# rvp-group/srrg2_proslam

Hardware: AMD Instinct MI355X
Metric: tracked frames/sec on KITTI-00 stereo (1241x376, ~2k kp); SE(3) vs ref (higher is better)
Workload: dtype u64 popcount (Hamming) + f32 (projection, Jacobians, 6x6 normal equations)

## Files before the change

srrg2_proslam_amd/csrc/align.hip:

```cpp
#include "prs_device.h"
#include "prs_host.h"
#include "prs_se3.h"

#include <math.h>
#include <string.h>

#include <type_traits>
#include <vector>

namespace prs {

constexpr int kAlignThreads = 256;
constexpr int kTerms        = 29;
constexpr uint32_t kNoneU32 = 0xffffffffu;
constexpr float kFltMax     = 3.402823466e+38f;

typedef unsigned int au32x4 __attribute__((ext_vector_type(4)));

struct AlignShared {
  float X[16];
  float A[16];
  float Sinv[16];
  float T[16];
  float Tprev[16];
// ... 383 lines not shown
  const double sx = (double) st[0], sy = (double) st[1];
  mean[0]          = (float) (sx / (16.0 * dn));
  mean[1]          = (float) (sy / (16.0 * dn));
  const double cxx = ((double) st[2] - sx * sx / dn) / dn / 256.0;
  const double cxy = ((double) st[3] - sx * sy / dn) / dn / 256.0;
  const double cyy = ((double) st[4] - sy * sy / dn) / dn / 256.0;
  const double half_diff = 0.5 * (cxx - cyy);
  double lambda          = 0.5 * (cxx + cyy) + sqrt(half_diff * half_diff + cxy * cxy);
  if (!(lambda > 0.0)) {
    lambda = 0.0;
  }
  double vx = lambda - cyy, vy = cxy;
  const double norm = sqrt(vx * vx + vy * vy);
  if (norm > 0.0) {
    vx = vx / norm;
    vy = vy / norm;
  } else {
    vx = cxx >= cyy ? 1.0 : 0.0;
    vy = cxx >= cyy ? 0.0 : 1.0;
  }
  normal[0] = (float) vx;
  normal[1] = (float) vy;
  return n < min_points || 3.0 * sqrt(lambda) < leaf_range;
}
__device__ __forceinline__ float kd_side(const KdNode& nd, const float x, const float y) {
  const float dx = x - nd.mx, dy = y - nd.my;
  return dx * nd.nx + dy * nd.ny;
}
__host__ __device__ __forceinline__ int kd_open_capacity(const int max_fixed) {
  return max_fixed / 5 + 4;
}

template <int T, bool SPLIT, int STYPE, int SLOTS = 4>
__global__ __launch_bounds__(T, SPLIT ? 6 : 1) void align_kernel(const AlignArgs g) {
  extern __shared__ __attribute__((aligned(16))) unsigned char smem[];
  const int tid   = threadIdx.x;
  const int lane  = tid & 63;
  const int wave  = tid >> 6;
  const int tid_hot = tid;
  constexpr bool kReuse = SPLIT && SLOTS == 4;
  const int frame = blockIdx.x;

  int nF = g.b.n_fixed[frame];
  int nM = g.b.n_moving[frame];
  nF     = nF < 0 ? 0 : (nF > g.b.fixed_stride ? g.b.fixed_stride : nF);
  nM     = nM < 0 ? 0 : (nM > g.b.moving_stride ? g.b.moving_stride : nM);
  const size_t fbase = (size_t) frame * (size_t) g.b.fixed_stride;
  const size_t mbase = (size_t) frame * (size_t) g.b.moving_stride;
  const float4* __restrict__ gfix = reinterpret_cast<const float4*>(g.b.fixed) + fbase;
  const float4* __restrict__ gmov = reinterpret_cast<const float4*>(g.b.moving) + mbase;
  const au32x4* __restrict__ gfd  = reinterpret_cast<const au32x4*>(g.b.fixed_desc + fbase * PRS_DESC_BYTES);
  const au32x4* __restrict__ gmd  = reinterpret_cast<const au32x4*>(g.b.moving_desc + mbase * PRS_DESC_BYTES);
  prs_corr* __restrict__ gcorr    = g.b.corr + fbase;
  prs_pcf_state* gstate           = g.b.state + frame;
  prs_align_result* gres          = g.b.result + frame;

  uint2* db           = reinterpret_cast<uint2*>(smem + g.off_db);
  uint16_t* inv       = reinterpret_cast<uint16_t*>(smem + g.off_inv);
  uint16_t* cellstart = reinterpret_cast<uint16_t*>(smem + g.off_cellstart);
  float4* cfix        = reinterpret_cast<float4*>(smem + g.off_cfix);
  float4* cmov        = reinterpret_cast<float4*>(smem + g.off_cmov);
  au32x4* fdesc       = reinterpret_cast<au32x4*>(smem + g.off_fdesc);
  au32x4* fdesc_hi    = fdesc + g.max_fixed;
  float2* fuv         = reinterpret_cast<float2*>(smem + g.off_fuv);
  uint32_t* bestkey   = reinterpret_cast<uint32_t*>(smem + g.off_best);
  uint32_t* second    = reinterpret_cast<uint32_t*>(smem + g.off_second);
  uint16_t* lut       = reinterpret_cast<uint16_t*>(smem + g.off_lut);
  constexpr int kSurvivors = SLOTS;
  uint16_t* surv      = reinterpret_cast<uint16_t*>(smem + g.off_surv) + kSurvivors * tid;
  float* terms        = reinterpret_cast<float*>(smem + g.off_terms);
  uint8_t* clsbuf     = smem + g.off_cls;
  AlignShared& sh     = *reinterpret_cast<AlignShared*>(smem + g.off_sh);
  const int R         = g.rows_table;
  const int stype     = STYPE >= 0 ? STYPE : g.f.search_type;
  const bool lattice  = stype != PRS_SEARCH_KDTREE;

  constexpr bool split_search = SPLIT;
  FrameCtl* ctl           = split_search ? g.ctl + frame : nullptr;
  if (split_search && (ctl->done || !ctl->need_search)) {
    return;
  }

  if (tid < 16) {
    sh.X[tid]     = g.b.X[(size_t) frame * 16 + tid];
    sh.T[tid]     = gstate->local_map_in_sensor[tid];
    sh.Tprev[tid] = gstate->local_map_in_sensor_previous[tid];
  }
  if (tid == 0) {
    sh.radius         = gstate->search_radius_pixels;
    sh.it             = gstate->current_iteration;
    sh.dd             = gstate->descriptor_distance;
    sh.kd_range       = gstate->database_leaf_range;
    sh.converged      = gstate->has_converged;
    sh.config_changed = gstate->config_changed;
    sh.num_recomputes = gstate->num_recomputes;
    sh.no_prune       = gstate->reserved & 1;
    sh.n_overflow     = 0;
    if constexpr (kReuse) {
      sh.q_tag  = (split_search && ctl->it_align != 0 && ctl->db_ready) ? ctl->q_tag : 0;
      sh.q_miss = 0;
    }
    sh.n_corr         = g.b.n_corr[frame];
    sh.flags          = 0;
    sh.error          = 0;
    sh.n_inl = sh.n_out = sh.n_inv = 0;
    sh.chi_in = sh.chi_tot = 0.0f;
    sh.mean_disp           = (split_search && ctl->it_align != 0) ? gres->mean_disparity : g.a.mean_disparity;
    sh.corr_changed        = 1;
    sh.have_terms          = 0;
    sh.have_cls            = 0;
    if (sh.n_corr < 0 || sh.n_corr > nF) {
      sh.n_corr = 0;
    }
    {
      float x[16], a16[16], si[16];
      const float* gx = g.b.X + (size_t) frame * 16;
#pragma unroll
      for (int i = 0; i < 16; ++i) {
        x[i] = gx[i];
      }
      se3_inverse(g.a.sensor_in_robot, si);
      pose_to_camera(g.a, si, x, a16);
#pragma unroll
      for (int i = 0; i < 16; ++i) {
        sh.Sinv[i] = si[i];
        sh.A[i]    = a16[i];
      }
    }
    if (nF > g.max_fixed) {
      sh.error = PRS_ERR_CAPACITY;
    }
  }
  for (int i = tid; i < 36; i += T) {
    sh.H[i] = 0.0f;
  }
  if (tid < 6) {
    sh.b[tid] = 0.0f;
  }
  bool db_built = false;
  if (split_search && lattice && g.rowcache && ctl->db_ready && ctl->it_align != 0 && nF <= g.max_fixed) {
    const uint4* __restrict__ img   = reinterpret_cast<const uint4*>(g.dbcache + (size_t) frame * g.db_blob);
    const au32x4* __restrict__ rows = g.rowcache + (size_t) frame * 2 * (size_t) g.max_fixed;
    uint4* dst      = reinterpret_cast<uint4*>(smem + g.off_db);
    const int n_img = (int) (g.db_blob >> 4);
    for (int i = tid; i < (n_img > nF ? n_img : nF); i += T) {
      uint4 a   = make_uint4(0u, 0u, 0u, 0u);
      au32x4 lo = {0u, 0u, 0u, 0u}, hi = {0u, 0u, 0u, 0u};
      if (i < n_img) {
        a = img[i];
      }
      if (i < nF) {
        lo = rows[i];
        hi = rows[g.max_fixed + i];
      }
      if (i < n_img) {
        dst[i] = a;
      }
      if (i < nF) {
        fdesc[i]    = lo;
        fdesc_hi[i] = hi;
      }
    }
    db_built = true;
  }
  __syncthreads();

  bool inputs_changed = g.b.inputs_changed ? (g.b.inputs_changed[frame] != 0) : true;
  if (split_search && ctl->it_align != 0) {
    inputs_changed = false;
  }
  if (inputs_changed && g.mode != PRS_MODE_LINEARIZE) {
    if (tid == 0) {
      sh.n_corr = 0;
    }
    __syncthreads();
  }

  const auto binds_disparity = [&]() {
    return g.mode != PRS_MODE_FINDER && (!split_search || ctl->it_align == 0) && g.a.factor_type == PRS_FACTOR_STEREO && g.a.enable_inverse_depth_weighting &&
           g.a.mean_disparity < 0.0f;
  };
  const auto bind_disparity = [&]() {
    for (int i = tid; i < nF; i += T) {
      const float4 c = gfix[i];
      terms[i]       = c.x - c.z;
    }
    __syncthreads();
    if (tid == 0) {
      sh.mean_disp = nF > 0 ? serial_float_sum(terms, nF) / (float) (size_t) nF : 0.0f;
    }
    __syncthreads();
  };
  if (!(split_search && lattice) && binds_disparity() && !sh.error) {
    bind_disparity();
  }

  if (g.mode != PRS_MODE_FINDER && !split_search && !sh.error) {
    for (int c = tid; c < sh.n_corr; c += T) {
      const prs_corr cr = gcorr[c];
      if (cr.fixed_idx < 0 || cr.fixed_idx >= nF || cr.moving_idx < 0 || cr.moving_idx >= nM) {
        sh.error = PRS_ERR_RANGE;
      } else {
        cfix[c] = gfix[cr.fixed_idx];
        cmov[c] = gmov[cr.moving_idx];
      }
    }
    __syncthreads();
  }

  enum { acc_finder = 0, acc_lin, acc_sum, acc_solve, acc_db, acc_search, acc_pass2, acc_filter, acc_commit };
  if (g.stamps && tid == 0) {
    for (int i = 0; i < 9; ++i) {
      sh.stamp_acc[i] = 0;
    }
    sh.stamp_mark = sh.stamp_sub = 0;
  }
#define SUB_MARK() do { if (g.stamps && tid == 0) { sh.stamp_sub = (unsigned long long) clock64(); } } while (0)
#define SUB_ACC(v) do { if (g.stamps && tid == 0) { const unsigned long long now_ = (unsigned long long) clock64(); sh.stamp_acc[v] += now_ - sh.stamp_sub; sh.stamp_sub = now_; } } while (0)
#define ALIGN_MARK() do { if (g.stamps && tid == 0) { sh.stamp_mark = (unsigned long long) clock64(); } } while (0)
#define ALIGN_ACC(v) do { if (g.stamps && tid == 0) { sh.stamp_acc[v] += (unsigned long long) clock64() - sh.stamp_mark; } } while (0)
  const int max_it = (g.mode == PRS_MODE_ALIGN && !sh.error) ? g.a.max_iterations + inlier_run_length(g.a) : (sh.error ? 0 : 1);
  if (split_search && sh.error && tid == 0) {
    ctl->done = 1;
  }
  int executed     = 0;
  int it_align     = 0;
  bool ran_inlier_phase = false;
  for (; it_align < max_it; ++it_align) {
    const bool inlier_run = g.mode == PRS_MODE_ALIGN && it_align >= g.a.max_iterations;
    if (g.mode == PRS_MODE_ALIGN && it_align == g.a.max_iterations) {
      if (sh.n_inl < g.a.min_num_inliers) {
        break;
      }
      ran_inlier_phase = true;
    }
    ++executed;
    ALIGN_MARK();
    if (g.mode != PRS_MODE_LINEARIZE && !inlier_run) {
      if (tid < 16) {
        sh.T[tid] = sh.A[tid];
      }
      __syncthreads();
      for (;;) {
        const bool reset = inputs_changed || sh.config_changed;
        __syncthreads();
        if (reset) {
          if (tid == 0) {
            if ((sh.radius == 0 && sh.dd == 0.0f) || sh.config_changed) {
              sh.radius = g.f.maximum_search_radius_pixels;
              sh.dd     = g.f.minimum_descriptor_distance;
            }
            if (sh.config_changed) {
              sh.no_prune = 0;
            }
            sh.converged = 0;
            sh.it        = 0;
            se3_identity(sh.Tprev);
            sh.config_changed = 0;
            sh.kd_range       = (float) sh.radius;
            if constexpr (kReuse) {
              sh.q_tag = 0;
            }
          }
          inputs_changed = false;
          db_built       = false;
          __syncthreads();
        }
        if (sh.error) {
          break;
        }

        if (tid == 0) {
          if (nF == 0 || nM == 0) {
            sh.flags |= PRS_WARN_EMPTY_INPUT;
          }
          sh.decision = kDecisionCommit;
          if (sh.converged) {
            sh.decision = kDecisionReturn;
          } else {
            float cam[16];
            se3_inverse(sh.T, cam);
            const unsigned long long k = g.f.number_of_solver_iterations_per_projection;
            if (k == 0 || sh.it % k == 0 || sh.it == 1) {
              se3_inverse(cam, sh.W);
              float delta[16], v6[6];
              se3_mul(cam, sh.Tprev, delta);
              t2tnq(delta, v6);
              sh.change_norm =
                sqrtf(((((v6[0] * v6[0] + v6[1] * v6[1]) + v6[2] * v6[2]) + v6[3] * v6[3]) + v6[4] * v6[4]) + v6[5] * v6[5]);
#pragma unroll
              for (int i = 0; i < 16; ++i) {
                sh.Tprev[i] = sh.T[i];
              }
              sh.n_projected = 0;
              sh.n_overflow  = 0;
              if constexpr (kReuse) {
                sh.q_miss = 0;
              }
              ++sh.num_recomputes;
            } else {
#pragma unroll
              for (int i = 0; i < 16; ++i) {
                sh.Tprev[i] = sh.T[i];
              }
              ++sh.it;
              sh.decision = kDecisionReturn;
            }
          }
        }
        __syncthreads();
        if (sh.decision == kDecisionReturn) {
          break;
        }

        SUB_MARK();
        const bool stage_rows = !split_search || !db_built;
        if (!db_built && split_search && g.dbcache && ctl->db_ready) {
          const uint4* src = reinterpret_cast<const uint4*>(g.dbcache + (size_t) frame * g.db_blob);
          uint4* dst       = reinterpret_cast<uint4*>(smem + g.off_db);
          for (int i = tid; i < (int) (g.db_blob >> 4); i += T) {
            dst[i] = src[i];
          }
          __syncthreads();
          db_built = true;
        }
        if (!db_built && !lattice) {
          const int tid = cold_copy(tid_hot), lane = tid & 63, wave = tid >> 6;
          (void) lane;
          (void) wave;
          KdNode* nodes        = reinterpret_cast<KdNode*>(db);
          uint16_t* order      = inv;
          short* kdhead        = reinterpret_cast<short*>(cellstart);
          uint16_t* leaf_start = cellstart + 2;
          const int node_cap   = (int) ((size_t) g.max_fixed * sizeof(uint2) / sizeof(KdNode));
          const int open_cap   = kd_open_capacity(g.max_fixed);
          const int min_points = g.f.minimum_number_of_points_per_cluster > 0 ? g.f.minimum_number_of_points_per_cluster : 10;
          unsigned long long* st = reinterpret_cast<unsigned long long*>(terms);
          int* cnt        = reinterpret_cast<int*>(st + (size_t) open_cap * 5);
          int* kind       = cnt + open_cap;
          int* child_open = kind + open_cap;
          int* par_cur    = child_open + open_cap;
          int* pcnt_cur   = par_cur + open_cap;
          int* par_next   = pcnt_cur + open_cap;
          int* pcnt_next  = par_next + open_cap;
          uint16_t* node_of = reinterpret_cast<uint16_t*>(pcnt_next + open_cap);
          uint16_t* leaf_of = node_of + g.max_fixed + 2;
          uint16_t* bucket  = leaf_of + g.max_fixed + 2;
          for (int i = tid; i < nF; i += T) {
            const float4 c = gfix[i];
            if (!(c.x > -32768.0f && c.x < 32768.0f && c.y > -32768.0f && c.y < 32768.0f)) {
              sh.error = PRS_ERR_RANGE;
            }
            node_of[i] = 0;
          }
          if (tid == 0) {
            sh.kd_nodes = sh.kd_leaves = 0;
            par_cur[0]  = -1;
            pcnt_cur[0] = -1;
            if (nF == 0) {
              kdhead[0]     = (short) ~0;
              sh.kd_leaves  = 1;
            }
          }
          __syncthreads();
          if (sh.error) {
            break;
          }
          int n_open = nF > 0 ? 1 : 0;
          while (n_open > 0) {
            for (int k = tid; k < n_open; k += T) {
#pragma unroll
              for (int j = 0; j < 5; ++j) {
                st[5 * k + j] = 0ull;
              }
              cnt[k] = 0;
            }
            if (tid == 0) {
              sh.kd_open_next = 0;
            }
            __syncthreads();
            for (int i = tid; i < nF; i += T) {
              const int k = node_of[i];
              if (k != 0xffff) {
                const float4 c     = gfix[i];
                const long long qx = __float2ll_rn(c.x * 16.0f), qy = __float2ll_rn(c.y * 16.0f);
                atomicAdd(&st[5 * k + 0], (unsigned long long) qx);
                atomicAdd(&st[5 * k + 1], (unsigned long long) qy);
                atomicAdd(&st[5 * k + 2], (unsigned long long) (qx * qx));
                atomicAdd(&st[5 * k + 3], (unsigned long long) (qx * qy));
                atomicAdd(&st[5 * k + 4], (unsigned long long) (qy * qy));
                atomicAdd(&cnt[k], 1);
              }
            }
            __syncthreads();
            for (int k = tid; k < n_open; k += T) {
              const int n = cnt[k];
              int code    = 0x7fffffff;
              if (n > 0) {
                const int P       = par_cur[k] < 0 ? -1 : (par_cur[k] & 0x3fffffff);
                const int side    = par_cur[k] < 0 ? 0 : ((par_cur[k] >> 30) & 1);
                const bool forced = pcnt_cur[k] == n;
                float mean[2], normal[2];
                bool leaf = kd_decide(reinterpret_cast<const long long*>(st + 5 * k), n, (double) sh.kd_range, min_points, mean, normal) || forced;
                int N     = -1;
                if (!leaf) {
                  N = atomicAdd(&sh.kd_nodes, 1);
                  const int c0 = atomicAdd(&sh.kd_open_next, 2);
                  if (N >= node_cap || N > 32767 || c0 + 2 > open_cap) {
                    sh.error = PRS_ERR_CAPACITY;
                    leaf     = true;
                  } else {
                    KdNode nd;
                    nd.mx = mean[0];
                    nd.my = mean[1];
                    nd.nx = normal[0];
                    nd.ny = normal[1];
                    nd.child[0] = nd.child[1] = (short) ~0;
                    nd.pad   = 0;
                    nodes[N] = nd;
                    child_open[k]     = c0;
                    par_next[c0]      = N;
                    par_next[c0 + 1]  = N | (1 << 30);
                    pcnt_next[c0]     = n;
                    pcnt_next[c0 + 1] = n;
                    code              = N;
                  }
                }
                if (leaf) {
                  code = ~atomicAdd(&sh.kd_leaves, 1);
                }
                if (P < 0) {
                  kdhead[0] = (short) code;
                } else if (forced) {
                  nodes[P].child[0] = nodes[P].child[1] = (short) code;
                } else {
                  nodes[P].child[side] = (short) code;
                }
              }
              kind[k] = code;
            }
            __syncthreads();
            if (sh.error) {
              break;
            }
            const int next_open = sh.kd_open_next;
            for (int i = tid; i < nF; i += T) {
              const int k = node_of[i];
              if (k != 0xffff) {
                const int code = kind[k];
                if (code < 0) {
                  leaf_of[i] = (uint16_t) ~code;
                  node_of[i] = 0xffff;
                } else {
                  const float4 c = gfix[i];
                  node_of[i]     = (uint16_t) (child_open[k] + (kd_side(nodes[code], c.x, c.y) < 0.0f ? 0 : 1));
                }
              }
            }
            n_open = next_open;
            {
              int* t0 = par_cur;
              par_cur = par_next;
              par_next = t0;
              t0       = pcnt_cur;
              pcnt_cur = pcnt_next;
              pcnt_next = t0;
            }
            __syncthreads();
          }
          if (sh.error) {
            break;
          }
          const int n_leaves = sh.kd_leaves;
          uint32_t* lh       = reinterpret_cast<uint32_t*>(st);
          for (int l = tid; l <= n_leaves; l += T) {
            lh[l] = 0;
          }
          __syncthreads();
          for (int i = tid; i < nF; i += T) {
            node_of[i] = (uint16_t) atomicAdd(&lh[leaf_of[i]], 1u);
          }
          __syncthreads();
          if (wave == 0) {
            const int n     = n_leaves + 1;
            const int chunk = (n + 63) >> 6;
            uint32_t sum    = 0;
            for (int j = 0; j < chunk; ++j) {
              const int r = lane * chunk + j;
              sum += r < n ? lh[r] : 0u;
            }
            uint32_t incl = sum;
#pragma unroll
            for (int d = 1; d < 64; d <<= 1) {
              const uint32_t o = __shfl_up(incl, d, 64);
              if (lane >= d) {
                incl += o;
              }
            }
            uint32_t run = incl - sum;
            for (int j = 0; j < chunk; ++j) {
              const int r = lane * chunk + j;
              if (r < n) {
                leaf_start[r] = (uint16_t) run;
                run += lh[r];
              }
            }
          }
          __syncthreads();
          for (int i = tid; i < nF; i += T) {
            bucket[leaf_start[leaf_of[i]] + node_of[i]] = (uint16_t) i;
          }
          __syncthreads();
          for (int i = tid; i < nF; i += T) {
            const int l0 = leaf_start[leaf_of[i]], l1 = leaf_start[leaf_of[i] + 1];
            int rank = 0;
            for (int j = l0; j < l1; ++j) {
              rank += bucket[j] < (uint16_t) i ? 1 : 0;
            }
            order[l0 + rank] = (uint16_t) i;
          }
          if (tid == 0) {
            kdhead[1] = (short) n_leaves;
          }
          __syncthreads();
          db_built = true;
          if (split_search && g.dbcache) {
            const uint4* src = reinterpret_cast<const uint4*>(smem + g.off_db);
            uint4* dst       = reinterpret_cast<uint4*>(g.dbcache + (size_t) frame * g.db_blob);
            for (int i = tid; i < (int) (g.db_blob >> 4); i += T) {
              dst[i] = src[i];
            }
            if (tid == 0) {
              ctl->db_ready = 1;
            }
          }
        }
        if (!db_built) {
          const int tid = cold_copy(tid_hot), lane = tid & 63, wave = tid >> 6;
          (void) lane;
          (void) wave;
          constexpr int kWaves = T / 64;
          static_assert(2 * kWaves <= 16, "AlignShared::wave_tot holds the wave totals of both scans");
          float* disp         = terms;
          uint32_t* hist_row  = reinterpret_cast<uint32_t*>(disp + g.max_fixed + 40);
          uint32_t* hist_cell = hist_row + R + 2;
          uint32_t* rowcol    = hist_cell + g.ncells + 2;
          int* dsum           = reinterpret_cast<int*>(rowcol + g.max_fixed);
          uint16_t* slot      = reinterpret_cast<uint16_t*>(dsum + 4);
          uint16_t* cslot     = slot + g.max_fixed + 2;
          uint16_t* bucket    = cslot + g.max_fixed + 2;
          uint16_t* rowfirst  = bucket + g.max_fixed + 2;
          const bool bind     = split_search && binds_disparity();
          for (int i = tid; i <= R; i += T) {
            hist_row[i] = 0;
          }
          for (int i = tid; i <= g.ncells; i += T) {
            hist_cell[i] = 0;
          }
          if (tid == 0) {
            dsum[0] = dsum[1] = dsum[2] = 0;
          }
          __syncthreads();
          int msum = 0, mabs = 0;
          bool inexact = false;
          for (int i = tid; i < nF; i += T) {
            const float4 c = gfix[i];
            if (bind) {
              const float d = c.x - c.z;
              const float q = d * 16.0f;
              const bool ok = __builtin_fabsf(q) < 1048576.0f && q == __builtin_rintf(q);
              const int m   = ok ? (int) q : 0;
              disp[i]       = d;
              msum += m;
              mabs += m < 0 ? -m : m;
              inexact = inexact || !ok;
            }
            if (c.x >= 0.0f && c.x < 32767.0f && c.y >= 0.0f && c.y < (float) R) {
              const int row = (int) (int16_t) c.y;
              const int col = (int) (int16_t) c.x;
              int cxi       = col >> g.cell_sx;
              cxi           = cxi < g.cell_ncx ? cxi : g.cell_ncx - 1;
              rowcol[i]     = ((uint32_t) row & 0xffffu) | ((uint32_t) col << 16);
              slot[i]       = (uint16_t) atomicAdd(&hist_row[row], 1u);
              cslot[i]      = (uint16_t) atomicAdd(&hist_cell[(row >> g.cell_sy) * g.cell_ncx + cxi], 1u);
            } else {
              sh.error = PRS_ERR_RANGE;
            }
          }
          if (bind) {
            const uint32_t wsum = wave_inclusive_scan_dpp((uint32_t) msum), wabs = wave_inclusive_scan_dpp((uint32_t) mabs);
            const bool winexact = __ballot(inexact) != 0ull;
            if (lane == 63) {
              atomicAdd(&dsum[0], (int) wsum);
              atomicAdd(&dsum[1], (int) wabs);
              if (winexact) {
                dsum[2] = 1;
              }
            }
          }
          __syncthreads();
          if (sh.error) {
            break;
          }
          {
            const int chunk_r = (R + T) / T, chunk_c = (g.ncells + T) / T;
            uint32_t sum_r = 0, sum_c = 0;
            for (int j = 0; j < chunk_r; ++j) {
              const int r = tid * chunk_r + j;
              sum_r += r <= R ? hist_row[r] : 0u;
            }
            for (int j = 0; j < chunk_c; ++j) {
              const int r = tid * chunk_c + j;
              sum_c += r <= g.ncells ? hist_cell[r] : 0u;
            }
            const uint32_t incl_r = wave_inclusive_scan_dpp(sum_r), incl_c = wave_inclusive_scan_dpp(sum_c);
            if (lane == 63) {
              sh.wave_tot[wave]          = (int) incl_r;
              sh.wave_tot[kWaves + wave] = (int) incl_c;
            }
            if (bind && tid == T - 64) {
              const bool exact = !dsum[2] && dsum[1] < (1 << 24);
              const float acc  = exact ? (float) dsum[0] * 0.0625f : serial_float_sum(disp, nF);
              sh.mean_disp     = nF > 0 ? acc / (float) (size_t) nF : 0.0f;
            }
            __syncthreads();
            uint32_t run_r = incl_r - sum_r, run_c = incl_c - sum_c;
#pragma unroll
            for (int w = 0; w < kWaves; ++w) {
              run_r += w < wave ? (uint32_t) sh.wave_tot[w] : 0u;
              run_c += w < wave ? (uint32_t) sh.wave_tot[kWaves + w] : 0u;
            }
            for (int j = 0; j < chunk_r; ++j) {
              const int r = tid * chunk_r + j;
              if (r <= R) {
                rowfirst[r] = (uint16_t) run_r;
                run_r += hist_row[r];
              }
            }
            for (int j = 0; j < chunk_c; ++j) {
              const int r = tid * chunk_c + j;
              if (r <= g.ncells) {
                cellstart[r] = (uint16_t) run_c;
                run_c += hist_cell[r];
              }
            }
          }
          __syncthreads();
          for (int i = tid; i < nF; i += T) {
            bucket[rowfirst[rowcol[i] & 0xffffu] + slot[i]] = (uint16_t) i;
          }
          __syncthreads();
          for (int i = tid; i < nF; i += T) {
            const uint32_t rc = rowcol[i];
            const int row = (int) (rc & 0xffffu), col = (int) (rc >> 16);
            const int s = rowfirst[row], e = rowfirst[row + 1];
            int rank = 0;
            for (int j = s; j < e; ++j) {
              rank += bucket[j] < (uint16_t) i ? 1 : 0;
            }
            const int canon = s + rank;
            int cxi         = col >> g.cell_sx;
            cxi             = cxi < g.cell_ncx ? cxi : g.cell_ncx - 1;
            db[cellstart[(row >> g.cell_sy) * g.cell_ncx + cxi] + cslot[i]] = make_uint2(rc, (uint32_t) i | ((uint32_t) canon << 16));
            inv[canon]                                                      = (uint16_t) i;
          }
          if (tid == 0) {
            db[nF] = make_uint2(0x7fff7fffu, 0xffffffffu);
          }
          __syncthreads();
          db_built = true;
          if (split_search && g.dbcache) {
            const uint4* src = reinterpret_cast<const uint4*>(smem + g.off_db);
            uint4* dst       = reinterpret_cast<uint4*>(g.dbcache + (size_t) frame * g.db_blob);
            for (int i = tid; i < (int) (g.db_blob >> 4); i += T) {
              dst[i] = src[i];
            }
            if (tid == 0) {
              ctl->db_ready = 1;
            }
          }
        }

        SUB_ACC(acc_db);
        const int rad = (int) sh.radius;
        {
          const int tid = cold_copy(tid_hot);
          for (int i = tid; i < nF; i += T) {
            bestkey[i] = kNoneU32;
            second[i]  = kNoneU32;
          }
          if (lattice) {
            if (stage_rows) {
              au32x4* rows = split_search && g.rowcache ? g.rowcache + (size_t) frame * 2 * (size_t) g.max_fixed : nullptr;
              for (int pos = tid; pos < nF; pos += T) {
                const int fi    = (int) (db[pos].y & 0xffffu);
                const au32x4 lo = gfd[2 * fi], hi = gfd[2 * fi + 1];
                fdesc[pos]      = lo;
                fdesc_hi[pos]   = hi;
                if (rows) {
                  rows[pos]               = lo;
                  rows[g.max_fixed + pos] = hi;
                }
              }
            }
          } else {
            for (int i = tid; i < 2 * nF; i += T) {
              (i & 1 ? fdesc_hi : fdesc)[i >> 1] = gfd[i];
            }
            for (int i = tid; i < nF; i += T) {
              const float4 c = gfix[i];
              fuv[i]         = make_float2(c.x, c.y);
            }
          }
          if (stype == PRS_SEARCH_CIRCLE) {
            for (int i = tid; i < 2 * rad + 1 && i < g.lut_cap; i += T) {
              const int h = i - rad;
              lut[i]      = (uint16_t) (isqrt_exact(rad * rad - h * h) + 1);
            }
          }
        }
        __syncthreads();
        SUB_ACC(acc_pass2);
        {
          const float W0 = sh.W[0], W1 = sh.W[1], W2 = sh.W[2], W3 = sh.W[3];
          const float W4 = sh.W[4], W5 = sh.W[5], W6 = sh.W[6], W7 = sh.W[7];
          const float W8 = sh.W[8], W9 = sh.W[9], W10 = sh.W[10], W11 = sh.W[11];
          const float cols = (float) g.f.projector.canvas_cols, rows = (float) g.f.projector.canvas_rows;
          const float max_dd = g.f.maximum_descriptor_distance;
          const float r2f    = (float) (sh.radius * sh.radius);
          const int rad2     = rad * rad;
          const int irrelevant = irrelevant_distance(sh.dd, g.f.maximum_distance_ratio_to_second_best);
          const int prune_at   = (lattice && irrelevant > 0 && irrelevant <= 54 && !g.no_prefilter && !sh.no_prune) ? irrelevant : 0;
          const bool circle_exact = rad < 8192 && R + rad < 32000 && (g.cell_ncx << g.cell_sx) + rad < 32000;
          int projected      = 0;
          const bool q_on   = kReuse && split_search && g.qcache != nullptr && prune_at > 0;
          const int q_tag   = q_on ? (prune_at | ((prune_at <= g.narrow_prefilter_limit ? 3 : 4) << 8)) : 0;
          const bool q_read = q_on && (sh.q_tag & 0xffff) == q_tag;
          au32x4* const qc  = q_on ? g.qcache + mbase : nullptr;
          if (kReuse && split_search && tid == 0) {
            sh.q_tag = (sh.q_tag & 0xffff) | (q_tag << 16);
          }
          auto query = [&](const int m, const float4 p, au32x4 q0, au32x4 q1, const au32x4 ent, auto first_pass_tag) {
            constexpr bool FIRST_PASS = decltype(first_pass_tag)::value;
// ... 239 lines not shown
                qc[m]               = au32x4{none, none, none, none};
              }
              if (bestk != kNoneU32) {
                cd.x = (lattice ? (uint32_t) inv[bestk & 0xffffu] : (bestk & 0xffffu)) | ((bestk >> 16) << 16);
                if (lattice && seck != kNoneU32) {
                  cd.y = (uint32_t) inv[seck & 0xffffu] | ((seck >> 16) << 16);
                }
              }
              auto emit = [&](const uint32_t c, const uint32_t tag) {
                const uint32_t f   = c & 0xffffu;
                const uint32_t key = ((c >> 16) << 17) | ((uint32_t) m << 1) | tag;
                const uint32_t old = atomicMin(&bestkey[f], key);
                if (old != kNoneU32) {
                  atomicMin(&second[f], (old > key ? old : key) >> 17);
                }
              };
              if (cd.x != kNoneU32) {
                emit(cd.x, 0u);
              }
              if (cd.y != kNoneU32) {
                emit(cd.y, 1u);
              }
            } else if (FIRST_PASS ? ent.y != 0u : q_on) {
              const uint32_t none = (uint32_t) cold_copy(0);
              qc[m]               = au32x4{none, none, none, none};
            }
          };
          constexpr int kPre = SPLIT ? 1 : 4;
          if constexpr (!kReuse) {
            for (int m0 = tid; m0 < nM; m0 += kPre * T) {
              float4 pre_p[kPre];
              au32x4 pre_q0[kPre], pre_q1[kPre];
#pragma unroll
              for (int qi = 0; qi < kPre; ++qi) {
                const int mm = m0 + qi * T < nM ? m0 + qi * T : m0;
                pre_p[qi]    = gmov[mm];
                pre_q0[qi]   = gmd[2 * mm];
                pre_q1[qi]   = gmd[2 * mm + 1];
              }
#pragma unroll
              for (int qi = 0; qi < kPre; ++qi) {
                const int m = m0 + qi * T;
                if (m >= nM) {
                  continue;
                }
                query(m, pre_p[qi], pre_q0[qi], pre_q1[qi], au32x4{0u, 0u, 0u, 0u}, std::false_type{});
              }
            }
          } else {
            static_assert(kPre == 1, "the search half fetches one query at a time");
            int n_query = nM;
            if (q_read) {
              constexpr int kQPre = 2;
              for (int m0 = tid; m0 < nM; m0 += kQPre * T) {
                float4 pre_p[kQPre];
                au32x4 pre_e[kQPre];
#pragma unroll
                for (int qi = 0; qi < kQPre; ++qi) {
                  const int mm = m0 + qi * T < nM ? m0 + qi * T : m0;
                  pre_p[qi]    = gmov[mm];
                  pre_e[qi]    = qc[mm];
                }
#pragma unroll
                for (int qi = 0; qi < kQPre; ++qi) {
                  const int m = m0 + qi * T;
                  if (m < nM) {
                    query(m, pre_p[qi], au32x4{0u, 0u, 0u, 0u}, au32x4{0u, 0u, 0u, 0u}, pre_e[qi], std::true_type{});
                  }
                }
              }
              __syncthreads();
              SUB_ACC(acc_lin);
              n_query = sh.q_miss;
            }
            for (int i = tid; i < n_query; i += T) {
              const int m = q_read ? (int) g.missq[mbase + (size_t) i] : i;
              query(m, gmov[m], gmd[2 * m], gmd[2 * m + 1], au32x4{0u, 0u, 0u, 0u}, std::false_type{});
            }
          }
          if (projected) {
            atomicAdd(&sh.n_projected, projected);
          }
        }
        __syncthreads();
        SUB_ACC(acc_search);
        const int f_tid = kReuse ? cold_copy(tid_hot) : tid, f_lane = kReuse ? (f_tid & 63) : lane, f_wave = kReuse ? (f_tid >> 6) : wave;
        {
          const int tid = f_tid, lane = f_lane, wave = f_wave;
          const float ratio = g.f.maximum_distance_ratio_to_second_best;
          const float dd    = sh.dd;
          int base          = 0;
          constexpr int kWaves = T / 64;
          static_assert(2 * kWaves <= 16, "AlignShared::wave_tot holds the wave totals of two chunks");
          for (int f0 = 0; f0 < nF; f0 += 2 * T) {
            if (f0 != 0) {
              __syncthreads();
            }
            bool acc[2];
            int pre[2];
#pragma unroll
            for (int k = 0; k < 2; ++k) {
              const int f = f0 + k * T + tid;
              acc[k]      = false;
              if (f < nF) {
                const uint32_t bk = bestkey[f];
                if (bk != kNoneU32) {
                  const float resp = (float) (bk >> 17);
                  const uint32_t s = second[f];
                  const float fs   = s == kNoneU32 ? kFltMax : (float) s;
                  acc[k] = resp < dd && resp / fs < ratio && (bk & 1u) == 0u;
                }
              }
              const unsigned long long bal = __ballot(acc[k]);
              pre[k]                       = __popcll(bal & ((1ull << lane) - 1ull));
              if (lane == 0) {
                sh.wave_tot[k * kWaves + wave] = __popcll(bal);
              }
            }
            __syncthreads();
            int wbase[2] = {0, 0};
            int run      = base;
#pragma unroll
            for (int j = 0; j < 2 * kWaves; ++j) {
              if (j == wave) {
                wbase[0] = run;
              }
              if (j == kWaves + wave) {
                wbase[1] = run;
              }
              run += sh.wave_tot[j];
            }
            base = run;
#pragma unroll
            for (int k = 0; k < 2; ++k) {
              const int f = f0 + k * T + tid;
              if (f < nF) {
                second[f] = acc[k] ? (uint32_t) (wbase[k] + pre[k]) : kNoneU32;
              }
            }
          }
          if (tid == 0) {
            sh.n_filtered = base;
          }
        }
        if (tid == 0) {
          if (sh.n_projected == 0) {
            sh.flags |= PRS_WARN_NO_PROJECTION;
          }
          if (8 * sh.n_overflow > sh.n_projected) {
            sh.no_prune = 1;
          }
          if (kReuse && split_search) {
            const int tag_now = sh.q_tag >> 16;
            if (tag_now != 0 && (sh.q_tag & 0xffff) == tag_now) {
              atomicAdd(&ctl->q_hits, sh.n_projected - sh.q_miss);
              atomicAdd(&ctl->q_misses, sh.q_miss);
            }
            sh.q_tag = tag_now;
          }
          const float matching_ratio = (float) sh.n_filtered / (float) (size_t) nF;
          sh.decision                = kDecisionCommit;
          if (matching_ratio < g.f.minimum_matching_ratio) {
            sh.flags |= PRS_WARN_LOW_RATIO;
            if (sh.radius < g.f.maximum_search_radius_pixels || sh.dd > g.f.minimum_descriptor_distance) {
              sh.radius = g.f.maximum_search_radius_pixels;
              sh.dd     = g.f.minimum_descriptor_distance;
              sh.flags |= PRS_WARN_RETRIED;
              if (matching_ratio == 0.0f) {
                sh.flags |= PRS_WARN_TRACK_LOST;
// ... 208 lines not shown
      break;
    }
  }

  if (!split_search) {
    __syncthreads();
  }
  if (g.mode == PRS_MODE_ALIGN && !split_search && g.a.keep_only_inlier_correspondences && sh.have_cls && !sh.error) {
    const int nc = sh.n_corr;
    int base     = 0;
    for (int c0 = 0; c0 < nc; c0 += T) {
      const int c     = c0 + tid;
      const bool keep = c < nc && clsbuf[c] == 0;
      prs_corr cr;
      if (keep) {
        cr = gcorr[c];
      }
      const unsigned long long bal = __ballot(keep);
      if (lane == 0) {
        sh.wave_tot[wave] = __popcll(bal);
      }
      __syncthreads();
      int pos = base + __popcll(bal & ((1ull << lane) - 1ull));
      for (int w = 0; w < T / 64; ++w) {
        pos += w < wave ? sh.wave_tot[w] : 0;
        base += sh.wave_tot[w];
      }
      if (keep) {
        gcorr[pos] = cr;
      }
      __syncthreads();
    }
    if (tid == 0) {
      sh.n_corr = base;
    }
    __syncthreads();
  }

  if (split_search && lattice && !db_built && binds_disparity() && sh.error != PRS_ERR_CAPACITY) {
    bind_disparity();
  }

  if (!split_search) {
    __syncthreads();
  }
  if (tid < 16) {
    if (!split_search) {
      g.b.X[(size_t) frame * 16 + tid] = sh.X[tid];
    }
    gstate->local_map_in_sensor[tid]          = sh.T[tid];
    gstate->local_map_in_sensor_previous[tid] = sh.Tprev[tid];
  }
  for (int i = tid; i < 36; i += T) {
    gres->H[i] = sh.H[i];
  }
  if (tid < 6) {
    gres->b[tid] = sh.b[tid];
  }
  if (tid == 0) {
    gstate->search_radius_pixels = sh.radius;
    gstate->current_iteration    = sh.it;
    gstate->descriptor_distance  = sh.dd;
    gstate->database_leaf_range  = sh.kd_range;
    gstate->has_converged        = sh.converged;
    gstate->config_changed       = sh.config_changed;
    gstate->num_recomputes       = sh.num_recomputes;
    gstate->reserved             = (gstate->reserved & ~1) | sh.no_prune;
    g.b.n_corr[frame]            = sh.n_corr;
    gres->chi_inliers            = sh.chi_in;
    gres->chi_total              = sh.chi_tot;
    gres->mean_disparity         = sh.mean_disp;
    gres->num_inliers            = sh.n_inl;
    gres->num_outliers           = sh.n_out;
    gres->num_invalid            = sh.n_inv;
    gres->num_correspondences    = sh.n_corr;
    gres->status                 = sh.n_inl >= g.a.min_num_inliers ? 1 : 0;
    gres->iterations             = g.mode == PRS_MODE_ALIGN ? (ran_inlier_phase ? max_it : g.a.max_iterations) : 1;
    gres->iterations_executed    = executed;
    gres->warnings               = sh.error ? sh.error : sh.flags;
    if (split_search) {
      ctl->flags |= sh.flags;
      ctl->need_search = 0;
      gres->warnings   = sh.error ? sh.error : ctl->flags;
      if constexpr (kReuse) {
        ctl->q_tag = sh.q_tag & 0xffff;
      }
    }
    if (g.stamps) {
      unsigned long long* st = g.stamps + (size_t) frame * 16;
      st[0] = 0;
      for (int i = 0; i < 9; ++i) {
        st[i + 1] = st[i] + sh.stamp_acc[i];
      }
    }
  }
}

constexpr int kGnThreads = 128;
constexpr int kGnSlots   = 8;

struct GnShared {
  float X[16], T[16], Tprev[16];
  float H[36], b[6];
  float chi_in, chi_tot;
  float fcnt[3];
  float pad0;
  float A[16];
  float Sinv[16];
  float wsum[32];
  unsigned long long it;
  int converged, need_search, n_inl, n_out, n_inv, stop, flags;
  int pose_ok;
  int wave_tot[4];
};
static_assert(offsetof(GnShared, b) == offsetof(GnShared, H) + 36 * sizeof(float) && offsetof(GnShared, chi_in) == offsetof(GnShared, b) + 6 * sizeof(float) &&
                offsetof(GnShared, chi_tot) == offsetof(GnShared, chi_in) + sizeof(float) && offsetof(GnShared, fcnt) == offsetof(GnShared, chi_tot) + sizeof(float),
              "the summed slots are written through GnShared::H");

__device__ __forceinline__ bool gn_advance(const prs_aligner_params& a, const int extra, int& it_align, bool fixed_point, const int n_inl) {
  const bool was_inlier_run = it_align >= a.max_iterations;
  ++it_align;
  if (fixed_point && !was_inlier_run && extra > 0) {
    it_align    = a.max_iterations;
    fixed_point = false;
  }
  if (fixed_point) {
    return true;
  }
  if (it_align == a.max_iterations && extra > 0) {
    return n_inl < a.min_num_inliers;
  }
  return it_align >= a.max_iterations + extra;
}

template <bool SHIPPED_FORMS = false, int PLAIN = 0>
__device__ __forceinline__ void gn_solve_wave(const AlignArgs& g, GnShared& sh, const int frame, const int nc, const int stid, const bool inlier_run) {
  const int lane = stid;
  if (sh.pose_ok) {
    const int rrow = lane < 6 ? lane : 5;
    const int blk  = rrow >= 3 ? 1 : 0;
    const int ci   = rrow - 3 * blk;
    const float* Yb = &sh.H[18 * blk];
    const float Ri0 = sh.A[ci], Ri1 = sh.A[4 + ci], Ri2 = sh.A[8 + ci];
    float o[6];
#pragma unroll
    for (int cb = 0; cb < 2; ++cb) {
      float v[3];
#pragma unroll
      for (int c = 0; c < 3; ++c) {
        v[c] = fmaf(Ri2, Yb[12 + 3 * cb + c], fmaf(Ri1, Yb[6 + 3 * cb + c], Ri0 * Yb[3 * cb + c]));
      }
#pragma unroll
      for (int j = 0; j < 3; ++j) {
        o[3 * cb + j] = fmaf(v[2], sh.A[8 + j], fmaf(v[1], sh.A[4 + j], v[0] * sh.A[j]));
      }
    }
    const float bb = fmaf(Ri2, sh.b[3 * blk + 2], fmaf(Ri1, sh.b[3 * blk + 1], Ri0 * sh.b[3 * blk]));
    __builtin_amdgcn_fence(__ATOMIC_RELEASE, "wavefront");
    __builtin_amdgcn_wave_barrier();
    __builtin_amdgcn_fence(__ATOMIC_ACQUIRE, "wavefront");
    if (lane < 6) {
      float2* hw = reinterpret_cast<float2*>(&sh.H[6 * rrow]);
      hw[0]      = make_float2(o[0], o[1]);
      hw[1]      = make_float2(o[2], o[3]);
      hw[2]      = make_float2(o[4], o[5]);
      sh.b[rrow] = bb;
// ... 982 lines not shown
```

Before: 1.957 million.

## Skip row sort when fixed keypoints are row-sorted; defer change-norm pose update

Adds a check during the lattice database build for whether fixed keypoints are already ordered by row. When they are, the row histogram, row scan, bucket scatter and per-row rank loop are skipped and the identity index is used as the canonical order. The change-norm and Tprev update move out of the serial tid-0 decision block to a thread that runs after the search. Other edits: skip the sensor-pose transform when there is no sensor, narrow the modulo to 32-bit, drop one barrier, and mark the frame done on error. The sortedness test reads the previous element's y field with a loose comparison, and removing the barrier after writing sh.T may introduce ordering risks.

```diff
diff --git a/srrg2_proslam_amd/csrc/align.hip b/srrg2_proslam_amd/csrc/align.hip
--- a/srrg2_proslam_amd/csrc/align.hip
+++ b/srrg2_proslam_amd/csrc/align.hip
@@ -489,7 +489,11 @@
   }
 
   if (tid < 16) {
-    sh.X[tid]     = g.b.X[(size_t) frame * 16 + tid];
+    const float x = g.b.X[(size_t) frame * 16 + tid];
+    sh.X[tid]     = x;
+    if (!g.a.with_sensor) {
+      sh.A[tid] = x;
+    }
     sh.T[tid]     = gstate->local_map_in_sensor[tid];
     sh.Tprev[tid] = gstate->local_map_in_sensor_previous[tid];
   }
@@ -519,7 +523,7 @@
     if (sh.n_corr < 0 || sh.n_corr > nF) {
       sh.n_corr = 0;
     }
-    {
+    if (g.a.with_sensor) {
       float x[16], a16[16], si[16];
       const float* gx = g.b.X + (size_t) frame * 16;
 #pragma unroll
@@ -601,6 +605,12 @@
   if (!(split_search && lattice) && binds_disparity() && !sh.error) {
     bind_disparity();
   }
+  const auto move_projection_pose = [&]() {
+    const int tid = cold_copy(tid_hot);
+    if (tid < 16) {
+      sh.Tprev[tid] = sh.T[tid];
+    }
+  };
 
   if (g.mode != PRS_MODE_FINDER && !split_search && !sh.error) {
     for (int c = tid; c < sh.n_corr; c += T) {
@@ -647,7 +657,6 @@
       if (tid < 16) {
         sh.T[tid] = sh.A[tid];
       }
-      __syncthreads();
       for (;;) {
         const bool reset = inputs_changed || sh.config_changed;
         __syncthreads();
@@ -687,18 +696,11 @@
           } else {
             float cam[16];
             se3_inverse(sh.T, cam);
-            const unsigned long long k = g.f.number_of_solver_iterations_per_projection;
-            if (k == 0 || sh.it % k == 0 || sh.it == 1) {
+            const unsigned long long k = g.f.number_of_solver_iterations_per_projection, it = sh.it;
+            const bool reproject = k == 0 || it <= 1 ||
+                                   (((it | k) >> 32) == 0 ? (uint32_t) it % (uint32_t) k == 0 : it % k == 0);
+            if (reproject) {
               se3_inverse(cam, sh.W);
-              float delta[16], v6[6];
-              se3_mul(cam, sh.Tprev, delta);
-              t2tnq(delta, v6);
-              sh.change_norm =
-                sqrtf(((((v6[0] * v6[0] + v6[1] * v6[1]) + v6[2] * v6[2]) + v6[3] * v6[3]) + v6[4] * v6[4]) + v6[5] * v6[5]);
-#pragma unroll
-              for (int i = 0; i < 16; ++i) {
-                sh.Tprev[i] = sh.T[i];
-              }
               sh.n_projected = 0;
               sh.n_overflow  = 0;
               if constexpr (kReuse) {
@@ -771,6 +773,7 @@
           }
           __syncthreads();
           if (sh.error) {
+            move_projection_pose();
             break;
           }
           int n_open = nF > 0 ? 1 : 0;
@@ -876,6 +879,7 @@
             __syncthreads();
           }
           if (sh.error) {
+            move_projection_pose();
             break;
           }
           const int n_leaves = sh.kd_leaves;
@@ -958,20 +962,18 @@
           uint16_t* bucket    = cslot + g.max_fixed + 2;
           uint16_t* rowfirst  = bucket + g.max_fixed + 2;
           const bool bind     = split_search && binds_disparity();
-          for (int i = tid; i <= R; i += T) {
-            hist_row[i] = 0;
-          }
           for (int i = tid; i <= g.ncells; i += T) {
             hist_cell[i] = 0;
           }
           if (tid == 0) {
-            dsum[0] = dsum[1] = dsum[2] = 0;
+            dsum[0] = dsum[1] = dsum[2] = dsum[3] = 0;
           }
           __syncthreads();
           int msum = 0, mabs = 0;
           bool inexact = false;
           for (int i = tid; i < nF; i += T) {
             const float4 c = gfix[i];
+            const float pv = reinterpret_cast<const float*>(gfix)[4 * (i > 0 ? i - 1 : 0) + 1];
             if (bind) {
               const float d = c.x - c.z;
               const float q = d * 16.0f;
@@ -988,8 +990,10 @@
               int cxi       = col >> g.cell_sx;
               cxi           = cxi < g.cell_ncx ? cxi : g.cell_ncx - 1;
               rowcol[i]     = ((uint32_t) row & 0xffffu) | ((uint32_t) col << 16);
-              slot[i]       = (uint16_t) atomicAdd(&hist_row[row], 1u);
               cslot[i]      = (uint16_t) atomicAdd(&hist_cell[(row >> g.cell_sy) * g.cell_ncx + cxi], 1u);
+              if (pv >= 0.0f && pv < (float) R && (int) (int16_t) pv > row) {
+                dsum[3] = 1;
+              }
             } else {
               sh.error = PRS_ERR_RANGE;
             }
@@ -1007,10 +1011,23 @@
           }
           __syncthreads();
           if (sh.error) {
+            move_projection_pose();
             break;
           }
+          const auto is_sorted = [&]() { return __builtin_amdgcn_readfirstlane(dsum[3]) == 0; };
+          if (!is_sorted()) {
+            for (int i = tid; i <= R; i += T) {
+              hist_row[i] = 0;
+            }
+            __syncthreads();
+            for (int i = tid; i < nF; i += T) {
+              slot[i] = (uint16_t) atomicAdd(&hist_row[rowcol[i] & 0xffffu], 1u);
+            }
+            __syncthreads();
+          }
           {
-            const int chunk_r = (R + T) / T, chunk_c = (g.ncells + T) / T;
+            const bool sorted = is_sorted();
+            const int chunk_r = sorted ? 0 : (R + T) / T, chunk_c = (g.ncells + T) / T;
             uint32_t sum_r = 0, sum_c = 0;
             for (int j = 0; j < chunk_r; ++j) {
               const int r = tid * chunk_r + j;
@@ -1020,7 +1037,7 @@
               const int r = tid * chunk_c + j;
               sum_c += r <= g.ncells ? hist_cell[r] : 0u;
             }
-            const uint32_t incl_r = wave_inclusive_scan_dpp(sum_r), incl_c = wave_inclusive_scan_dpp(sum_c);
+            const uint32_t incl_r = sorted ? 0u : wave_inclusive_scan_dpp(sum_r), incl_c = wave_inclusive_scan_dpp(sum_c);
             if (lane == 63) {
               sh.wave_tot[wave]          = (int) incl_r;
               sh.wave_tot[kWaves + wave] = (int) incl_c;
@@ -1053,19 +1070,25 @@
             }
           }
           __syncthreads();
-          for (int i = tid; i < nF; i += T) {
-            bucket[rowfirst[rowcol[i] & 0xffffu] + slot[i]] = (uint16_t) i;
-          }
-          __syncthreads();
+          const bool sorted = is_sorted();
+          if (!sorted) {
+            for (int i = tid; i < nF; i += T) {
+              bucket[rowfirst[rowcol[i] & 0xffffu] + slot[i]] = (uint16_t) i;
+            }
+            __syncthreads();
+          }
           for (int i = tid; i < nF; i += T) {
             const uint32_t rc = rowcol[i];
             const int row = (int) (rc & 0xffffu), col = (int) (rc >> 16);
-            const int s = rowfirst[row], e = rowfirst[row + 1];
-            int rank = 0;
-            for (int j = s; j < e; ++j) {
-              rank += bucket[j] < (uint16_t) i ? 1 : 0;
-            }
-            const int canon = s + rank;
+            int canon     = i;
+            if (!sorted) {
+              const int s = rowfirst[row], e = rowfirst[row + 1];
+              int rank = 0;
+              for (int j = s; j < e; ++j) {
+                rank += bucket[j] < (uint16_t) i ? 1 : 0;
+              }
+              canon = s + rank;
+            }
             int cxi         = col >> g.cell_sx;
             cxi             = cxi < g.cell_ncx ? cxi : g.cell_ncx - 1;
             db[cellstart[(row >> g.cell_sy) * g.cell_ncx + cxi] + cslot[i]] = make_uint2(rc, (uint32_t) i | ((uint32_t) canon << 16));
@@ -1471,9 +1494,21 @@
             atomicAdd(&sh.n_projected, projected);
           }
         }
+        if (cold_copy(tid_hot) == T - 64) {
+          float cam[16], delta[16], v6[6];
+          se3_inverse(sh.T, cam);
+          se3_mul(cam, sh.Tprev, delta);
+          t2tnq(delta, v6);
+          sh.change_norm =
+            sqrtf(((((v6[0] * v6[0] + v6[1] * v6[1]) + v6[2] * v6[2]) + v6[3] * v6[3]) + v6[4] * v6[4]) + v6[5] * v6[5]);
+#pragma unroll
+          for (int i = 0; i < 16; ++i) {
+            sh.Tprev[i] = sh.T[i];
+          }
+        }
         __syncthreads();
         SUB_ACC(acc_search);
-        const int f_tid = kReuse ? cold_copy(tid_hot) : tid, f_lane = kReuse ? (f_tid & 63) : lane, f_wave = kReuse ? (f_tid >> 6) : wave;
+        const int f_tid = SPLIT ? cold_copy(tid_hot) : tid, f_lane = kReuse ? (f_tid & 63) : lane, f_wave = kReuse ? (f_tid >> 6) : wave;
         {
           const int tid = f_tid, lane = f_lane, wave = f_wave;
           const float ratio = g.f.maximum_distance_ratio_to_second_best;
@@ -1848,6 +1883,9 @@
       ctl->flags |= sh.flags;
       ctl->need_search = 0;
       gres->warnings   = sh.error ? sh.error : ctl->flags;
+      if (sh.error) {
+        ctl->done = 1;
+      }
       if constexpr (kReuse) {
         ctl->q_tag = sh.q_tag & 0xffff;
       }
```

Result: no change. 1.971 million, median of 6 (+0.7%).
